# um-dsrg/Super-Resolution-Meta-Attention-Networks

Hardware: AMD Instinct MI355X
Metric: LR-patches/sec (128x128x3, x4) fwd+bwd (higher is better)
Workload: dtype f32

## Files before the change

### super-resolution-meta-attention-networks_amd/csrc/conv3x3_mfma.hip

```cpp
#include "sisr_common.h"
#include "ca_gate.h"
#include <string.h>
#include <stdlib.h>
#include <type_traits>

#define TH 4
#define TW 32
#define HALO_H (TH + 2)
#define HALO_W (TW + 2)
#define HALO_ITEMS (HALO_H * HALO_W * 16)
#define STAGE_ITERS ((HALO_ITEMS + 255) / 256)

struct ConvParams {
  const float* x;
  View xv;
  float* y;
  View yv;
  const float* res;
  const float* mask;
  const float* w;
  const float* bias;
  const float* in_scale;
  const float* in_shift;
  const float* out_scale;
// ... 878 lines not shown
          if (AFFINE) t = t * s4 + t4;
          if (GATE) {
            t = sisr_mul_add4(t, s4, u[r][k]);
            if (rown && cok && col >= 1 && col <= TW)
              sisr_buf_store4(t, ro_, (unsigned)(min(max(gw, 0), W - 1) * (int)p.xv.sW + c4 * 4) * 4u, ro);
          }
          if (!interior) t = sisr_keep_if(t, rok && cok);
          *reinterpret_cast<f32x4*>(lds + r * (HALO_W * 64) + col * 64 + ((c4 ^ (col & 15)) << 2)) = t;
        }
    }
  };

  unsigned aoff[4];
#pragma unroll
  for (int j = 0; j < 4; ++j) {
    const int col = 2 * n + j;
    aoff[j] = (unsigned)(2 * mb * (HALO_W * 64) + col * 64 + ((q ^ (col & 15)) << 2));
  }

  if (t_begin < t_end) {
    halo_regs_t v;
    issue(v, t_begin, 0, HHv);
    commit(v, t_begin);
  }
  __syncthreads();
  for (int tile = t_begin; tile < t_end; tile += t_step) {
    const bool has_next = tile + t_step < t_end;
    int b, h0, w0;
    decode(tile, b, h0, w0);
#define W4_LOAD_B(t) \
  sisr_buf_load4(rw, boff, (unsigned)((((((t) >> 5) * 4 + (((t) >> 1) & 3)) * 4 + (((t) >> 3) & 3)) * 4096) + ((t) & 1) * 256))
    f32x4 bq[8];
#pragma unroll
    for (int t = 0; t < 6; ++t) bq[t] = W4_LOAD_B(t);
    f32x4 y[2][2][2];
    f32x4 acc[4][2];
    f32x4 raw[4], rr[4], av[2][4];
    halo_regs_t v;
    auto read_half = [&](int s, int hc) {
      const int xr = s >> 2, G = s & 3;
      const int ra = xr == 0 ? 0 : (xr == 3 ? 3 : 2), rb = xr == 0 ? 2 : 1;
#pragma unroll
      for (int jj = 0; jj < 2; ++jj) {
        const float* base = lds + (aoff[2 * hc + jj] ^ (unsigned)(G << 4));
        raw[2 * jj] = *reinterpret_cast<const f32x4*>(base + ra * (HALO_W * 64));
        raw[2 * jj + 1] = *reinterpret_cast<const f32x4*>(base + rb * (HALO_W * 64));
      }
    };
    auto rows_half = [&](int s, int hc) {
      const int xr = s >> 2;
#pragma unroll
      for (int jj = 0; jj < 2; ++jj) {
        const f32x4 da = raw[2 * jj], db = raw[2 * jj + 1];
        rr[2 * hc + jj] = xr == 0 ? da - db : (xr == 1 ? db + da : (xr == 2 ? da - db : db - da));
      }
    };
    auto cols_step = [&](int s) {
      f32x4* a = av[s & 1];
      a[0] = rr[0] - rr[2];
      a[1] = rr[1] + rr[2];
      a[2] = rr[2] - rr[1];
      a[3] = rr[1] - rr[3];
    };
    read_half(0, 0);
    rows_half(0, 0);
    read_half(0, 1);
    rows_half(0, 1);
    cols_step(0);
    __builtin_amdgcn_sched_barrier(0);
#pragma unroll
    for (int s = 0; s < 16; ++s) {
      const int xr = s >> 2, G = s & 3;
      if (s == 12 && has_next) issue(v, tile + t_step, 0, 3);
      if (s == 14 && has_next) issue(v, tile + t_step, 3, HHv);
      if (s + 1 < 16) read_half(s + 1, 0);
#pragma unroll
      for (int xc = 0; xc < 4; ++xc) {
        const f32x4 a = av[s & 1][xc];
        f32x4 bb[2];
#pragma unroll
        for (int nb = 0; nb < 2; ++nb) {
          const int t = (s * 4 + xc) * 2 + nb;
          bb[nb] = bq[t & 7];
        }
#pragma unroll
        for (int e = 0; e < 4; ++e)
#pragma unroll
          for (int nb = 0; nb < 2; ++nb) {
            const f32x4 c = (G | e) ? acc[xc][nb] : (f32x4){0.f, 0.f, 0.f, 0.f};
            acc[xc][nb] = __builtin_amdgcn_mfma_f32_16x16x4f32(a[e], bb[nb][e], c, 0, 0, 0);
          }
#pragma unroll
        for (int nb = 0; nb < 2; ++nb) {
          const int t = (s * 4 + xc) * 2 + nb;
          if (t + 6 < 128) bq[(t + 6) & 7] = W4_LOAD_B(t + 6);
        }
        if (s + 1 < 16) {
          if (xc == 1) {
            rows_half(s + 1, 0);
            read_half(s + 1, 1);
          }
          if (xc == 2) rows_half(s + 1, 1);
          if (xc == 3) cols_step(s + 1);
        }
        __builtin_amdgcn_sched_barrier(0);
      }
      if (G == 3) {
#pragma unroll
        for (int nb = 0; nb < 2; ++nb) {
          const f32x4 t0 = acc[0][nb] + acc[1][nb] + acc[2][nb];
          const f32x4 t1 = acc[1][nb] - acc[2][nb] - acc[3][nb];
          if (xr == 0) { y[nb][0][0] = t0; y[nb][0][1] = t1; }
          if (xr == 1) { y[nb][0][0] += t0; y[nb][0][1] += t1; y[nb][1][0] = t0; y[nb][1][1] = t1; }
          if (xr == 2) { y[nb][0][0] += t0; y[nb][0][1] += t1; y[nb][1][0] -= t0; y[nb][1][1] -= t1; }
          if (xr == 3) { y[nb][1][0] -= t0; y[nb][1][1] -= t1; }
#pragma unroll
          for (int i = 0; i < (xr == 0 ? 1 : 2); ++i) asm volatile("" : "+v"(y[nb][i][0]), "+v"(y[nb][i][1]));
        }
      }
    }
#undef W4_LOAD_B
    __syncthreads();
    if (has_next) commit(v, tile + t_step);
    {
      const bool scaled = p.out_scale != nullptr || p.alpha != 1.0f;
      const sisr_rsrc_t ry = sisr_rsrc(p.y + (long)b * p.yv.sB);
      const sisr_rsrc_t rmk = sisr_rsrc(MASK ? p.mask + (long)b * p.yv.sB : p.y);
      const sisr_rsrc_t rrs = sisr_rsrc(RES ? p.res + (long)b * p.yv.sB : p.y);
      const sisr_rsrc_t rdt = sisr_rsrc(DOT ? p.dot + (long)b * p.yv.sB : p.y);
      float gsum[2];
#pragma unroll
      for (int nb = 0; nb < 2; ++nb) {
        const int con = co + 16 * nb;
        float os = p.alpha;
        if (p.out_scale) os *= p.out_scale[(long)b * 64 + con];
        float mk[2][2][4], rs[2][2][4], dt[2][2][4];
#pragma unroll
        for (int i = 0; i < 2; ++i)
#pragma unroll
          for (int j = 0; j < 2; ++j)
#pragma unroll
            for (int r = 0; r < 4; ++r) {
              const int row = min(h0 + 2 * mb + i, H - 1), col = min(w0 + 8 * q + 2 * r + j, W - 1);
              const unsigned vo = (unsigned)(col * (int)p.yv.sW + con) * 4u, so = (unsigned)(row * (int)p.yv.sH) * 4u;
              if (MASK) mk[i][j][r] = sisr_buf_load1(rmk, vo, so);
              if (RES) rs[i][j][r] = sisr_buf_load1(rrs, vo, so);
              if (DOT) dt[i][j][r] = sisr_buf_load1(rdt, vo, so);
            }
        float gs = 0.f;
#pragma unroll
        for (int i = 0; i < 2; ++i)
#pragma unroll
          for (int j = 0; j < 2; ++j)
#pragma unroll
            for (int r = 0; r < 4; ++r) {
              float a = y[nb][i][j][r] + bv[nb];
              if (p.relu) a = fmaxf(a, 0.f);
              if (scaled) a *= os;
              if (MASK) a = mk[i][j][r] > 0.f ? a : 0.f;
              if (RES) a += rs[i][j][r];
              const int row = h0 + 2 * mb + i, col = w0 + 8 * q + 2 * r + j;
              if (row < H && col < W) {
                sisr_buf_store1(a, ry, (unsigned)(col * (int)p.yv.sW + con) * 4u, (unsigned)(row * (int)p.yv.sH) * 4u);
                gs = DOT ? __builtin_fmaf(a, dt[i][j][r], gs) : gs + a;
              }
            }
        gs += __shfl_xor(gs, 16);
        gsum[nb] = gs + __shfl_xor(gs, 32);
      }
      if (p.gap && q == 0) {
        const long parts = (long)p.tiles_w * ((H + 3) / 4) * 2;
        const int th = h0 / THv, tw = w0 / TW;
#pragma unroll
        for (int nb = 0; nb < 2; ++nb) p.gap[(((long)b * parts) + (th * p.tiles_w + tw) * 2 + mb) * 64 + co + 16 * nb] = gsum[nb];
      }
    }
    __syncthreads();
  }
}

typedef __bf16 bf16x8 __attribute__((ext_vector_type(8)));

__device__ __forceinline__ u32x4 sisr_pack_bf16x8(f32x4 a, f32x4 b) {
  bf16x8 r;
  r[0] = (__bf16)a[0]; r[1] = (__bf16)a[1]; r[2] = (__bf16)a[2]; r[3] = (__bf16)a[3];
  r[4] = (__bf16)b[0]; r[5] = (__bf16)b[1]; r[6] = (__bf16)b[2]; r[7] = (__bf16)b[3];
  return __builtin_bit_cast(u32x4, r);
}

__device__ __forceinline__ bf16x8 sisr_buf_load_bf16x8(sisr_rsrc_t r, unsigned voff_bytes, unsigned soff_bytes) {
  return __builtin_bit_cast(bf16x8, __builtin_amdgcn_raw_buffer_load_b128(r, (int)voff_bytes, (int)soff_bytes, 0));
}

#define BH_PIX 128
#define BE_LD 68

template <bool AFFINE, bool MASK, bool RES, bool GATE = false, bool DOT = false>
__global__ __launch_bounds__(256, 3) void conv3x3_c64_bf16_kernel(ConvParams p) {
  extern __shared__ __attribute__((aligned(16))) unsigned char ldsb[];
  const int tid = threadIdx.x, lane = tid & 63, wave = tid >> 6;
  const int q = blockIdx.y;
  int bid;
  {
    const unsigned nb = gridDim.x, xcd = blockIdx.x & 7, idx = blockIdx.x >> 3;
    const unsigned qn = nb >> 3, rn = nb & 7;
    bid = (int)((xcd < rn ? xcd * (qn + 1) : rn * (qn + 1) + (xcd - rn) * qn) + idx);
  }
  const int tw = bid % p.tiles_w;
  bid /= p.tiles_w;
  const int th = bid % p.tiles_h;
  const int b = bid / p.tiles_h;
  const int h0 = th * TH, w0 = tw * TW;
  const int ph = __builtin_amdgcn_readfirstlane(wave >> 1), ch = __builtin_amdgcn_readfirstlane(wave & 1);
  const int n = lane & 31, hh = lane >> 5;
  const int H = p.H, W = p.W;
  const int co = ch * 32 + n;
  const int Cout = p.cout_chunks * 64;

  const float bv = p.bias ? p.bias[co * p.bias_n + q * p.bias_q] : 0.f;
// ... 1853 lines not shown
```

### super-resolution-meta-attention-networks_amd/csrc/diag.hip

```cpp
#include "sisr_common.h"

template <bool RAND>
__global__ __launch_bounds__(256) void mfma_peak_kernel(int iters, float* __restrict__ out,
                                                        unsigned long long* __restrict__ clk) {
  f32x16 acc0 = {0}, acc1 = {0};
  float a = threadIdx.x * 1e-3f, b = 1.0f + blockIdx.x * 1e-6f;
  float ra[4], rb[4];
  if (RAND) {
    unsigned h = (blockIdx.x * 256u + threadIdx.x) * 2654435761u + 12345u;
#pragma unroll
    for (int e = 0; e < 4; ++e) {
      h = h * 1664525u + 1013904223u;
      ra[e] = (float)(int)h * (1.0f / 2147483648.0f);
      h = h * 1664525u + 1013904223u;
      rb[e] = (float)(int)h * (1.0f / 2147483648.0f);
    }
  }
  const unsigned long long t0 = __builtin_amdgcn_s_memtime();
  const unsigned long long r0 = __builtin_amdgcn_s_memrealtime();
  for (int i = 0; i < iters; ++i) {
#pragma unroll
    for (int e = 0; e < 4; ++e) {
      acc0 = __builtin_amdgcn_mfma_f32_32x32x2f32(RAND ? ra[e] : a, RAND ? rb[e] : b, acc0, 0, 0, 0);
      acc1 = __builtin_amdgcn_mfma_f32_32x32x2f32(RAND ? rb[e] : b, RAND ? ra[3 - e] : a, acc1, 0, 0, 0);
    }
    if (!RAND) a += 1e-7f;
  }
  const unsigned long long t1 = __builtin_amdgcn_s_memtime();
  const unsigned long long r1 = __builtin_amdgcn_s_memrealtime();
  float s = 0.f;
#pragma unroll
  for (int r = 0; r < 16; ++r) s += acc0[r] + acc1[r];
  out[(long)blockIdx.x * 256 + threadIdx.x] = s;
  if (blockIdx.x == 0 && threadIdx.x == 0) {
    clk[0] = t1 - t0;
    clk[1] = r1 - r0;
  }
}

extern "C" int sisr_diag_mfma_peak(int blocks, int iters, float* out, unsigned long long* clk, void* stream) {
  if (blocks <= 0 || iters == 0 || !out || !clk) return SISR_ERR_ARG;
  if (iters > 0)
    hipLaunchKernelGGL(mfma_peak_kernel<false>, dim3(blocks), dim3(256), 0, (hipStream_t)stream, iters, out, clk);
  else
    hipLaunchKernelGGL(mfma_peak_kernel<true>, dim3(blocks), dim3(256), 0, (hipStream_t)stream, -iters, out, clk);
  return sisr_check_launch();
}

template <int KIND, int COUNT>
__global__ __launch_bounds__(256) void mfma_fill_kernel(int iters, float* __restrict__ out, const float* __restrict__ src,
                                                        unsigned long long* __restrict__ clk) {
  __shared__ __attribute__((aligned(16))) float lds[256 * 4 + 64];
  f32x16 acc0 = {0}, acc1 = {0};
  float a = threadIdx.x * 1e-3f, b = 1.0f + blockIdx.x * 1e-6f;
  float f0 = a, f1 = b;
  unsigned u0 = threadIdx.x, u1 = blockIdx.x;
  unsigned s0 = blockIdx.x;
  f32x4 q0 = {0.f, 0.f, 0.f, 0.f};
  unsigned long long w0 = threadIdx.x;
  const unsigned lofs = threadIdx.x * 16;
  const float* gp = src + threadIdx.x * 4;
  float* op = out + (long)blockIdx.x * 256 + threadIdx.x;
  lds[threadIdx.x] = a;
  __syncthreads();
  const unsigned long long t0 = __builtin_amdgcn_s_memtime();
  const unsigned long long r0 = __builtin_amdgcn_s_memrealtime();
  for (int i = 0; i < iters; ++i) {
#pragma unroll
    for (int e = 0; e < 8; ++e) {
      if (e & 1) acc1 = __builtin_amdgcn_mfma_f32_32x32x2f32(b, a, acc1, 0, 0, 0);
      else acc0 = __builtin_amdgcn_mfma_f32_32x32x2f32(a, b, acc0, 0, 0, 0);
#pragma unroll
      for (int k = 0; k < (COUNT + 7 - e) / 8; ++k) {
        if (KIND == 1) asm volatile("v_add_f32 %0, %0, %1" : "+v"(f0) : "v"(f1));
        if (KIND == 2) asm volatile("v_and_b32 %0, %0, %1" : "+v"(u0) : "v"(u1));
        if (KIND == 3) asm volatile("s_add_u32 %0, %0, 1" : "+s"(s0) : : "scc");
        if (KIND == 4) asm volatile("ds_read_b128 %0, %1" : "=v"(q0) : "v"(lofs));
        if (KIND == 5) asm volatile("global_load_dwordx4 %0, %1, off" : "=v"(q0) : "v"(gp));
        if (KIND == 6) asm volatile("ds_write_b128 %0, %1" : : "v"(lofs), "v"(q0));
        if (KIND == 7) asm volatile("global_store_dword %0, %1, off" : : "v"(op), "v"(f0));
        if (KIND == 8) asm volatile("v_mov_b32 %0, %1" : "=v"(u0) : "v"(u1));
        if (KIND == 9) asm volatile("s_nop 0");
        if (KIND == 10) asm volatile("v_pk_add_f32 %0, %0, %0" : "+v"(w0));
        if (KIND == 11) asm volatile("v_lshl_add_u64 %0, %0, 0, %0" : "+v"(w0));
        if (KIND == 12) asm volatile("global_load_dwordx4 %0, %1, %2" : "=v"(q0) : "v"(lofs), "s"(src));
      }
    }
    if ((KIND == 4 || KIND == 6) && (i & 3) == 3) asm volatile("s_waitcnt lgkmcnt(0)" ::: "memory");
    if ((KIND == 5 || KIND == 7 || KIND == 12) && (i & 3) == 3 && COUNT <= 8) asm volatile("s_waitcnt vmcnt(0)" ::: "memory");
    if ((KIND == 5 || KIND == 7 || KIND == 12) && (i & 1) == 1 && COUNT == 16) asm volatile("s_waitcnt vmcnt(0)" ::: "memory");
    if ((KIND == 5 || KIND == 7 || KIND == 12) && COUNT == 32) asm volatile("s_waitcnt vmcnt(0)" ::: "memory");
  }
  asm volatile("s_waitcnt vmcnt(0) lgkmcnt(0)" ::: "memory");
  const unsigned long long t1 = __builtin_amdgcn_s_memtime();
  const unsigned long long r1 = __builtin_amdgcn_s_memrealtime();
  float s = f0 + (float)u0 + (float)s0 + q0[0] + q0[3] + (float)(unsigned)w0;
#pragma unroll
  for (int r = 0; r < 16; ++r) s += acc0[r] + acc1[r];
  *op = s;
  if (blockIdx.x == 0 && threadIdx.x == 0) {
    clk[0] = t1 - t0;
    clk[1] = r1 - r0;
  }
}

extern "C" int sisr_diag_mfma_fill(int blocks, int iters, int kind, int count, float* out, const float* src,
                                   unsigned long long* clk, void* stream) {
  if (blocks <= 0 || iters <= 0 || !out || !src || !clk) return SISR_ERR_ARG;
#define FILL(K, C) \
  if (kind == K && count == C) { hipLaunchKernelGGL((mfma_fill_kernel<K, C>), dim3(blocks), dim3(256), 0, (hipStream_t)stream, iters, out, src, clk); return sisr_check_launch(); }
#define FILLK(K) FILL(K, 8) FILL(K, 16) FILL(K, 32)
  FILL(1, 0)
  FILLK(1) FILLK(2) FILLK(3) FILLK(4) FILLK(5) FILLK(6) FILLK(7) FILLK(8) FILLK(9) FILLK(10) FILLK(11) FILLK(12)
#undef FILLK
#undef FILL
  return SISR_ERR_UNSUPPORTED;
}
```

### super-resolution-meta-attention-networks_amd/csrc/sisr_common.h

```cpp
#pragma once
#include <hip/hip_runtime.h>
#include <stdint.h>

typedef float f32x4 __attribute__((ext_vector_type(4)));
typedef float f32x16 __attribute__((ext_vector_type(16)));

struct View {
  long sB, sH, sW;
  long chi, clo;
  int cdiv;
  __host__ __device__ long chunk(int q) const { return (long)(q / cdiv) * chi + (long)(q % cdiv) * clo; }
};

typedef unsigned u32x4 __attribute__((ext_vector_type(4)));
__device__ __forceinline__ f32x4 sisr_keep_if(f32x4 t, bool ok) {
  const unsigned m = ok ? 0xffffffffu : 0u;
  u32x4 b = __builtin_bit_cast(u32x4, t);
  b &= (u32x4){m, m, m, m};
  return __builtin_bit_cast(f32x4, b);
}

__device__ __forceinline__ f32x4 sisr_mul_add4(f32x4 a, f32x4 b, f32x4 c) {
#pragma clang fp contract(off)
  const f32x4 p = a * b;
  return p + c;
}

typedef __amdgpu_buffer_rsrc_t sisr_rsrc_t;
__device__ __forceinline__ sisr_rsrc_t sisr_rsrc(const void* base) {
  return __builtin_amdgcn_make_buffer_rsrc(const_cast<void*>(base), 0, (int)0xffffffffu, 0x00020000);
}
__device__ __forceinline__ f32x4 sisr_buf_load4(sisr_rsrc_t r, unsigned voff_bytes, unsigned soff_bytes) {
  return __builtin_bit_cast(f32x4, __builtin_amdgcn_raw_buffer_load_b128(r, (int)voff_bytes, (int)soff_bytes, 0));
}
__device__ __forceinline__ float sisr_buf_load1(sisr_rsrc_t r, unsigned voff_bytes, unsigned soff_bytes) {
  return __builtin_bit_cast(float, __builtin_amdgcn_raw_buffer_load_b32(r, (int)voff_bytes, (int)soff_bytes, 0));
}
__device__ __forceinline__ void sisr_buf_store4(f32x4 v, sisr_rsrc_t r, unsigned voff_bytes, unsigned soff_bytes) {
  __builtin_amdgcn_raw_buffer_store_b128(__builtin_bit_cast(u32x4, v), r, (int)voff_bytes, (int)soff_bytes, 0);
}
__device__ __forceinline__ void sisr_buf_store1(float v, sisr_rsrc_t r, unsigned voff_bytes, unsigned soff_bytes) {
  __builtin_amdgcn_raw_buffer_store_b32(__builtin_bit_cast(unsigned, v), r, (int)voff_bytes, (int)soff_bytes, 0);
}

#define SISR_OK 0
#define SISR_ERR_ARG (-1)
#define SISR_ERR_ALIGN (-2)
#define SISR_ERR_LAUNCH (-3)
#define SISR_ERR_UNSUPPORTED (-4)

static inline int sisr_check_launch() {
  hipError_t e = hipGetLastError();
  return e == hipSuccess ? SISR_OK : SISR_ERR_LAUNCH - (int)e * 16;
}
#define SISR_ALLOW_LDS(kernel, bytes)                                                                       \
  do {                                                                                                      \
    static bool done_ = false;                                                                              \
    if (!done_) {                                                                                           \
      (void)hipFuncSetAttribute(reinterpret_cast<const void*>(kernel),                                      \
                                hipFuncAttributeMaxDynamicSharedMemorySize, (int)(bytes));                  \
      done_ = true;                                                                                         \
    }                                                                                                       \
  } while (0)

static inline bool sisr_aligned16(const void* p) { return (reinterpret_cast<uintptr_t>(p) & 15) == 0; }
```

### super-resolution-meta-attention-networks_amd/csrc/wgrad3x3_mfma.hip

```cpp
#include "sisr_common.h"
#include <string.h>
#include <stdlib.h>

#define WT_H 8
#define WT_W 32
#define WH_H (WT_H + 2)
#define WH_W (WT_W + 2)
#define WSTR 32
#define X_ITEMS (WH_H * WH_W * 8)
#define X_ITERS ((X_ITEMS + 255) / 256)
#define Y_ITEMS (WT_H * WT_W * 8)
#define Y_ITERS (Y_ITEMS / 256)
#define LDS_X (WH_H * WH_W * WSTR)
#define LDS_Y (WT_H * WT_W * WSTR)
#define SLAB (9 * 16 * 64)
#define WG_MAX_UNITS 64

struct WgradParams {
  const float* x;
  View xv;
  const float* dy;
  View yv;
  const float* dy_scale;
  const float* dy_shift;
// ... 352 lines not shown
            for (int t = 0; t < 9; ++t) an[t] = xn[((t / 3) * WH_W + (t % 3)) * 64];
          }
          __builtin_amdgcn_sched_barrier(0);
#pragma unroll
          for (int t = 0; t < 9; ++t) acc[t] = __builtin_amdgcn_mfma_f32_32x32x2f32(av[t], bv, acc[t], 0, 0, 0);
          __builtin_amdgcn_sched_barrier(0);
          bv = bn;
#pragma unroll
          for (int t = 0; t < 9; ++t) av[t] = an[t];
        }
        xa = xn;
        yb = yn;
      }
    }
    __syncthreads();
    if (has_next) {
      commit(tile + t_step);
      __syncthreads();
    }
  }

  {
    float* out = p.slabs + ((long)blockIdx.x * ((long)gridDim.y * 4) + pair * 4 + cih * 2 + coh) * SLAB;
#pragma unroll
    for (int t = 0; t < 9; ++t)
#pragma unroll
      for (int r = 0; r < 16; ++r) out[(t * 16 + r) * 64 + lane] = acc[t][r];
  }
  if (do_bias) {
    __syncthreads();
    float* red = lds;
    *reinterpret_cast<f32x4*>(red + tid * 8) = bsa;
    *reinterpret_cast<f32x4*>(red + tid * 8 + 4) = bsb;
    __syncthreads();
    if (tid < 64) {
      const int cc8 = tid >> 3, e = tid & 7;
      float s = 0.f;
      for (int k = 0; k < 32; ++k) s += red[(k * 8 + cc8) * 8 + e];
      p.bias_slabs[((long)blockIdx.x * p.cout_chunks + cq) * 64 + tid] = s;
    }
  }
}

__global__ __launch_bounds__(256, 1) void wgrad3x3_c64_full_kernel(WgradParams p) { wgrad3x3_c64_full_body(p); }
__global__ __launch_bounds__(256, 1) void wgrad3x3_c64_full_batch_kernel(WgradBatch bt) { wgrad3x3_c64_full_body(bt.job[blockIdx.z]); }
__global__ __launch_bounds__(256, 1) void wgrad3x3_c64_full_geo_kernel(WgradParams p) { wgrad3x3_c64_full_body<true>(p); }

#define W4_TH 4
#define W4_HH (W4_TH + 2)
#define W4G_X (W4_HH * WH_W * 64)
#define W4G_Y (W4_TH * WT_W * 64)
#define W4G_LDS ((W4G_X + W4G_Y) * 4)

__global__ __launch_bounds__(256, 1) void wgrad3x3_c64_w4_kernel(WgradParams p) {
  extern __shared__ __attribute__((aligned(16))) float lds[];
  float* const ldx = lds;
  float* const ldy = lds + W4G_X;
  const int tid = threadIdx.x, lane = tid & 63, wave = tid >> 6;
  const int pair = blockIdx.y;
  const int cq = pair % p.cout_chunks, cc = pair / p.cout_chunks;
  const int cih = __builtin_amdgcn_readfirstlane(wave >> 1), coh = __builtin_amdgcn_readfirstlane(wave & 1);
  const int i = lane & 31, kk = lane >> 5;
  const int H = p.H, W = p.W;
  const bool do_bias = p.bias_slabs && cc == 0;
  const bool affine = p.dy_scale != nullptr || p.dy_shift != nullptr;
  const int Cout = p.cout_chunks * 64;

  f32x16 acc[16];
#pragma unroll
  for (int t = 0; t < 16; ++t) acc[t] = (f32x16){0};
  f32x4 bsa = {0.f, 0.f, 0.f, 0.f}, bsb = bsa;

  const int tiles_w = p.tiles_w, tiles_h = (H + W4_TH - 1) / W4_TH;
  const int tiles_per_img = tiles_w * tiles_h;
  const int total = tiles_per_img * p.B;
  int t_begin = blockIdx.x, t_end = total, t_step = p.S;
  if ((p.S & 7) == 0) {
    const int xcd = blockIdx.x & 7, idx = blockIdx.x >> 3, per = (total + 7) >> 3;
    t_begin = xcd * per + idx;
    t_end = min(total, (xcd + 1) * per);
    t_step = p.S >> 3;
  }
  struct Stage {
    f32x4 x[W4_HH][2];
    f32x4 xe[2];
    f32x4 y[W4_TH][2];
  };
  Stage st;
  const int c8 = tid & 7, pcol = tid >> 3;
  const int eidx = tid % 96, er = eidx >> 4, eside = (eidx >> 3) & 1, ec8 = eidx & 7;
  auto decode = [&](int tile, int& b, int& h0, int& w0) {
    b = tile / tiles_per_img;
    const int tr = tile - b * tiles_per_img;
    const int th = tr / tiles_w;
    h0 = th * W4_TH;
    w0 = (tr - th * tiles_w) * WT_W;
  };
  auto issue = [&](int tile) {
    int b, h0, w0;
    decode(tile, b, h0, w0);
    const sisr_rsrc_t rx = sisr_rsrc(p.x + (long)b * p.xv.sB + p.xv.chunk(cc));
    const sisr_rsrc_t ry = sisr_rsrc(p.dy + (long)b * p.yv.sB + p.yv.chunk(cq));
    const unsigned vx = (unsigned)(min(w0 + pcol, W - 1) * (int)p.xv.sW + c8 * 8) * 4u;
    const unsigned vy = (unsigned)(min(w0 + pcol, W - 1) * (int)p.yv.sW + c8 * 8) * 4u;
#pragma unroll
    for (int r = 0; r < W4_HH; ++r) {
      const unsigned so = (unsigned)(min(max(h0 - 1 + r, 0), H - 1) * (int)p.xv.sH) * 4u;
      st.x[r][0] = sisr_buf_load4(rx, vx, so);
      st.x[r][1] = sisr_buf_load4(rx, vx + 16u, so);
    }
    {
      const int gwe = min(max(eside ? w0 + WT_W : w0 - 1, 0), W - 1);
      const unsigned ve = (unsigned)(min(max(h0 - 1 + er, 0), H - 1) * (int)p.xv.sH + gwe * (int)p.xv.sW + ec8 * 8) * 4u;
      st.xe[0] = sisr_buf_load4(rx, ve, 0u);
      st.xe[1] = sisr_buf_load4(rx, ve + 16u, 0u);
    }
#pragma unroll
    for (int r = 0; r < W4_TH; ++r) {
      const unsigned so = (unsigned)(min(h0 + r, H - 1) * (int)p.yv.sH) * 4u;
      st.y[r][0] = sisr_buf_load4(ry, vy, so);
      st.y[r][1] = sisr_buf_load4(ry, vy + 16u, so);
    }
  };
  auto commit = [&](int tile) {
    int b, h0, w0;
    decode(tile, b, h0, w0);
    const bool interior = h0 >= 1 && h0 + W4_TH + 1 <= H && w0 >= 1 && w0 + WT_W + 1 <= W;
    const bool okc = w0 + pcol < W;
    if (!interior) {
#pragma unroll
      for (int r = 0; r < W4_HH; ++r) {
        const int gh = h0 - 1 + r;
        const bool ok = gh >= 0 && gh < H && okc;
        st.x[r][0] = sisr_keep_if(st.x[r][0], ok);
        st.x[r][1] = sisr_keep_if(st.x[r][1], ok);
      }
      const int gwe = eside ? w0 + WT_W : w0 - 1, ghe = h0 - 1 + er;
      const bool oke = ghe >= 0 && ghe < H && gwe >= 0 && gwe < W;
      st.xe[0] = sisr_keep_if(st.xe[0], oke);
      st.xe[1] = sisr_keep_if(st.xe[1], oke);
    }
    float* lx = ldx + (pcol + 1) * 64 + c8 * 8;
#pragma unroll
    for (int r = 0; r < W4_HH; ++r) {
      *reinterpret_cast<f32x4*>(lx + r * (WH_W * 64)) = st.x[r][0];
      *reinterpret_cast<f32x4*>(lx + r * (WH_W * 64) + 4) = st.x[r][1];
    }
    if (tid < 96) {
      float* le = ldx + (er * WH_W + (eside ? WH_W - 1 : 0)) * 64 + ec8 * 8;
      *reinterpret_cast<f32x4*>(le) = st.xe[0];
      *reinterpret_cast<f32x4*>(le + 4) = st.xe[1];
    }
    if (affine) {
      f32x4 s4a = {1.f, 1.f, 1.f, 1.f}, s4b = s4a, t4a = {0.f, 0.f, 0.f, 0.f}, t4b = t4a;
      if (p.dy_scale) {
        const float* sp = p.dy_scale + (long)b * Cout + cq * 64 + c8 * 8;
        s4a = *reinterpret_cast<const f32x4*>(sp);
        s4b = *reinterpret_cast<const f32x4*>(sp + 4);
      }
      if (p.dy_shift) {
        const float* tp = p.dy_shift + (long)b * Cout + cq * 64 + c8 * 8;
        t4a = *reinterpret_cast<const f32x4*>(tp);
        t4b = *reinterpret_cast<const f32x4*>(tp + 4);
      }
#pragma unroll
      for (int r = 0; r < W4_TH; ++r) {
        st.y[r][0] = st.y[r][0] * s4a + t4a;
        st.y[r][1] = st.y[r][1] * s4b + t4b;
      }
    }
    if (!interior) {
#pragma unroll
      for (int r = 0; r < W4_TH; ++r) {
        const bool ok = okc && h0 + r < H;
        st.y[r][0] = sisr_keep_if(st.y[r][0], ok);
        st.y[r][1] = sisr_keep_if(st.y[r][1], ok);
      }
    }
    float* ly = ldy + pcol * 64 + c8 * 8;
#pragma unroll
    for (int r = 0; r < W4_TH; ++r) {
      *reinterpret_cast<f32x4*>(ly + r * (WT_W * 64)) = st.y[r][0];
      *reinterpret_cast<f32x4*>(ly + r * (WT_W * 64) + 4) = st.y[r][1];
    }
    if (do_bias) {
#pragma unroll
      for (int r = 0; r < W4_TH; ++r) {
        bsa += st.y[r][0];
        bsb += st.y[r][1];
      }
    }
  };

  const float* const xl = ldx + kk * (2 * 64) + cih * 32 + i;
  const float* const yl = ldy + kk * (2 * 64) + coh * 32 + i;
  struct Raw {
    float d[4][4], y[2][2];
  };
  auto fetch = [&](int ks, Raw& rw) {
    const int br = ks >> 3, bc = ks & 7;
#pragma unroll
    for (int r = 0; r < 4; ++r)
#pragma unroll
      for (int j = 0; j < 4; ++j) rw.d[r][j] = xl[((2 * br + r) * WH_W + 4 * bc + j) * 64];
#pragma unroll
    for (int r = 0; r < 2; ++r)
#pragma unroll
      for (int j = 0; j < 2; ++j) rw.y[r][j] = yl[((2 * br + r) * WT_W + 4 * bc + j) * 64];
  };
  auto transform = [&](const Raw& rw, float (&V)[16], float (&M)[16]) {
    float rr[4][4];
#pragma unroll
    for (int j = 0; j < 4; ++j) {
      rr[0][j] = rw.d[0][j] - rw.d[2][j];
      rr[1][j] = rw.d[1][j] + rw.d[2][j];
      rr[2][j] = rw.d[2][j] - rw.d[1][j];
      rr[3][j] = rw.d[1][j] - rw.d[3][j];
    }
#pragma unroll
    for (int xr = 0; xr < 4; ++xr) {
      V[xr * 4 + 0] = rr[xr][0] - rr[xr][2];
      V[xr * 4 + 1] = rr[xr][1] + rr[xr][2];
      V[xr * 4 + 2] = rr[xr][2] - rr[xr][1];
      V[xr * 4 + 3] = rr[xr][1] - rr[xr][3];
    }
    float ry[4][2];
#pragma unroll
    for (int j = 0; j < 2; ++j) {
      ry[0][j] = rw.y[0][j];
      ry[1][j] = rw.y[0][j] + rw.y[1][j];
      ry[2][j] = rw.y[0][j] - rw.y[1][j];
      ry[3][j] = rw.y[1][j];
    }
#pragma unroll
    for (int xr = 0; xr < 4; ++xr) {
      M[xr * 4 + 0] = ry[xr][0];
      M[xr * 4 + 1] = ry[xr][0] + ry[xr][1];
      M[xr * 4 + 2] = ry[xr][0] - ry[xr][1];
      M[xr * 4 + 3] = ry[xr][1];
    }
  };

  float V[2][16], M[2][16];
  auto step_order = [&]() {
#pragma unroll
    for (int t = 0; t < 2; ++t) {
      __builtin_amdgcn_sched_group_barrier(0x008, 1, 0);
      __builtin_amdgcn_sched_group_barrier(0x100, 5, 0);
    }
    __builtin_amdgcn_sched_group_barrier(0x008, 2, 0);
#pragma unroll
    for (int t = 4; t < 15; ++t) {
      __builtin_amdgcn_sched_group_barrier(0x008, 1, 0);
      __builtin_amdgcn_sched_group_barrier(0x002, 4, 0);
    }
    __builtin_amdgcn_sched_group_barrier(0x008, 1, 0);
  };
  if (t_begin < t_end) {
    issue(t_begin);
    commit(t_begin);
    __syncthreads();
    Raw rw;
    fetch(0, rw);
    transform(rw, V[0], M[0]);
  }
  for (int tile = t_begin; tile < t_end; tile += t_step) {
    const bool has_next = tile + t_step < t_end;
    if (has_next) issue(tile + t_step);
#pragma unroll
    for (int ks = 0; ks < 15; ++ks) {
      const int cur = ks & 1, nxt = cur ^ 1;
      Raw rw;
      fetch(ks + 1, rw);
#pragma unroll
      for (int t = 0; t < 16; ++t)
        acc[t] = __builtin_amdgcn_mfma_f32_32x32x2f32(V[cur][t], M[cur][t], acc[t], 0, 0, 0);
      transform(rw, V[nxt], M[nxt]);
      step_order();
    }
    __syncthreads();
    if (has_next) commit(tile + t_step);
#pragma unroll
    for (int t = 0; t < 8; ++t) acc[t] = __builtin_amdgcn_mfma_f32_32x32x2f32(V[1][t], M[1][t], acc[t], 0, 0, 0);
    __builtin_amdgcn_sched_barrier(0);
    __syncthreads();
    {
      Raw rw;
      fetch(0, rw);
#pragma unroll
      for (int t = 8; t < 16; ++t) acc[t] = __builtin_amdgcn_mfma_f32_32x32x2f32(V[1][t], M[1][t], acc[t], 0, 0, 0);
      transform(rw, V[0], M[0]);
      __builtin_amdgcn_sched_group_barrier(0x008, 1, 0);
      __builtin_amdgcn_sched_group_barrier(0x100, 10, 0);
      __builtin_amdgcn_sched_group_barrier(0x008, 2, 0);
#pragma unroll
      for (int t = 0; t < 5; ++t) {
        __builtin_amdgcn_sched_group_barrier(0x008, 1, 0);
        __builtin_amdgcn_sched_group_barrier(0x002, 9, 0);
      }
    }
  }

  {
    float* out = p.slabs + ((long)blockIdx.x * ((long)gridDim.y * 4) + pair * 4 + cih * 2 + coh) * SLAB;
    auto fold = [](float u0, float u1, float u2, float u3, float& f0, float& f1, float& f2) {
      const float h = 0.5f * (u1 + u2);
      f0 = u0 + h;
      f1 = 0.5f * (u1 - u2);
      f2 = h - u3;
    };
#pragma unroll
    for (int r = 0; r < 16; ++r) {
      float rw[3][4];
#pragma unroll
      for (int xc = 0; xc < 4; ++xc) fold(acc[xc][r], acc[4 + xc][r], acc[8 + xc][r], acc[12 + xc][r], rw[0][xc], rw[1][xc], rw[2][xc]);
#pragma unroll
      for (int kh = 0; kh < 3; ++kh) {
        float g0, g1, g2;
        fold(rw[kh][0], rw[kh][1], rw[kh][2], rw[kh][3], g0, g1, g2);
        out[((kh * 3 + 0) * 16 + r) * 64 + lane] = g0;
        out[((kh * 3 + 1) * 16 + r) * 64 + lane] = g1;
        out[((kh * 3 + 2) * 16 + r) * 64 + lane] = g2;
      }
    }
  }
  if (do_bias) {
    __syncthreads();
    float* red = lds;
    *reinterpret_cast<f32x4*>(red + tid * 8) = bsa;
    *reinterpret_cast<f32x4*>(red + tid * 8 + 4) = bsb;
    __syncthreads();
    if (tid < 64) {
      const int cc8 = tid >> 3, e = tid & 7;
      float s = 0.f;
      for (int k = 0; k < 32; ++k) s += red[(k * 8 + cc8) * 8 + e];
      p.bias_slabs[((long)blockIdx.x * p.cout_chunks + cq) * 64 + tid] = s;
    }
  }
}

typedef __bf16 bf16x4 __attribute__((ext_vector_type(4)));
typedef __bf16 bf16x8 __attribute__((ext_vector_type(8)));
typedef bf16x4 __attribute__((address_space(3))) * lds_bf16x4_ptr;
#define BW_PIX 128
#define BW_X_BYTES (WH_H * WH_W * BW_PIX)
#define BW_Y_BYTES (WT_H * WT_W * BW_PIX)

__device__ __forceinline__ u32x4 wg_pack_bf16x8(f32x4 a, f32x4 b) {
  bf16x8 r;
  r[0] = (__bf16)a[0]; r[1] = (__bf16)a[1]; r[2] = (__bf16)a[2]; r[3] = (__bf16)a[3];
  r[4] = (__bf16)b[0]; r[5] = (__bf16)b[1]; r[6] = (__bf16)b[2]; r[7] = (__bf16)b[3];
  return __builtin_bit_cast(u32x4, r);
}

__device__ __forceinline__ bf16x8 wg_tr_frag(const unsigned char* base, unsigned off0, unsigned off1) {
  const bf16x4 lo = __builtin_amdgcn_ds_read_tr16_b64_v4bf16((lds_bf16x4_ptr)(base + off0));
  const bf16x4 hi = __builtin_amdgcn_ds_read_tr16_b64_v4bf16((lds_bf16x4_ptr)(base + off1));
  return __builtin_shufflevector(lo, hi, 0, 1, 2, 3, 4, 5, 6, 7);
}

template <bool X16, bool Y16>
static __device__ __forceinline__ void wgrad3x3_c64_bf16_body(const WgradParams& p, unsigned* stamp = nullptr) {
  extern __shared__ __attribute__((aligned(16))) unsigned char ldsb[];
  unsigned char* ldx = ldsb;
  unsigned char* ldy = ldsb + BW_X_BYTES;
  const int tid = threadIdx.x, lane = tid & 63, wave = tid >> 6;
  const int pair = blockIdx.y;
  const int cq = pair % p.cout_chunks, cc = pair / p.cout_chunks;
  const int cih = __builtin_amdgcn_readfirstlane(wave >> 1), coh = __builtin_amdgcn_readfirstlane(wave & 1);
  const int H = p.H, W = p.W;
  const bool do_bias = p.bias_slabs && cc == 0;
  const int Cout = p.cout_chunks * 64;

  f32x16 acc[9];
#pragma unroll
  for (int t = 0; t < 9; ++t) acc[t] = (f32x16){0};
  f32x4 bsa = {0.f, 0.f, 0.f, 0.f}, bsb = bsa;

  unsigned aoff[3][2], yoff[2];
  {
    const int g = lane >> 4, qq = (lane >> 2) & 3, pp = lane & 3;
    const int chunk = (g & 1) * 2 + (pp >> 1), sub = (pp & 1) * 8;
#pragma unroll
    for (int rd = 0; rd < 2; ++rd) {
      const int pix = 8 * (g >> 1) + 4 * rd + qq;
      yoff[rd] = pix * BW_PIX + (((coh * 4 + chunk) ^ (((pix >> 1) & 1) << 2)) << 4) + sub;
// ... 1104 lines not shown
```

Baseline: 119.2.

## Use packed v_pk_add_f32 for Winograd transforms and reschedule wgrad interleaving

Replaces scalar f32 add/sub in the conv3x3 Winograd input and output transforms with packed v_pk_add_f32 inline asm, halving the VALU instruction count. The wgrad kernel's input transform is rewritten on f32x2 pairs using op_sel/neg modifiers, and explicit sched barriers interleave the transform ops between individual MFMAs. The channel-to-thread mapping of the global and LDS staging changes to strided halves, with the bias reduction indexing updated to match. Diagnostic microbenchmarks for packed-add throughput alongside MFMA are added. Inline asm volatile may constrain compiler scheduling, and the remapping risks correctness errors if any index is missed.

After: 123.5, median of 6. +3.6%, better.

```diff
diff --git a/super-resolution-meta-attention-networks_amd/csrc/conv3x3_mfma.hip b/super-resolution-meta-attention-networks_amd/csrc/conv3x3_mfma.hip
--- a/super-resolution-meta-attention-networks_amd/csrc/conv3x3_mfma.hip
+++ b/super-resolution-meta-attention-networks_amd/csrc/conv3x3_mfma.hip
@@ -954,15 +954,15 @@
 #pragma unroll
       for (int jj = 0; jj < 2; ++jj) {
         const f32x4 da = raw[2 * jj], db = raw[2 * jj + 1];
-        rr[2 * hc + jj] = xr == 0 ? da - db : (xr == 1 ? db + da : (xr == 2 ? da - db : db - da));
+        rr[2 * hc + jj] = xr == 0 ? sisr_pk4_sub(da, db) : (xr == 1 ? sisr_pk4_add(db, da) : (xr == 2 ? sisr_pk4_sub(da, db) : sisr_pk4_sub(db, da)));
       }
     };
     auto cols_step = [&](int s) {
       f32x4* a = av[s & 1];
-      a[0] = rr[0] - rr[2];
-      a[1] = rr[1] + rr[2];
-      a[2] = rr[2] - rr[1];
-      a[3] = rr[1] - rr[3];
+      a[0] = sisr_pk4_sub(rr[0], rr[2]);
+      a[1] = sisr_pk4_add(rr[1], rr[2]);
+      a[2] = sisr_pk4_sub(rr[2], rr[1]);
+      a[3] = sisr_pk4_sub(rr[1], rr[3]);
     };
     read_half(0, 0);
     rows_half(0, 0);
@@ -1008,14 +1008,19 @@
         __builtin_amdgcn_sched_barrier(0);
       }
       if (G == 3) {
+        f32x4 t0[2], t1[2];
+#pragma unroll
+        for (int nb = 0; nb < 2; ++nb) t0[nb] = sisr_pk4_add(sisr_pk4_add(acc[0][nb], acc[1][nb]), acc[2][nb]);
+#pragma unroll
+        for (int nb = 0; nb < 2; ++nb) t1[nb] = sisr_pk4_sub(acc[1][nb], acc[2][nb]);
+#pragma unroll
+        for (int nb = 0; nb < 2; ++nb) t1[nb] = sisr_pk4_sub(t1[nb], acc[3][nb]);
 #pragma unroll
         for (int nb = 0; nb < 2; ++nb) {
-          const f32x4 t0 = acc[0][nb] + acc[1][nb] + acc[2][nb];
-          const f32x4 t1 = acc[1][nb] - acc[2][nb] - acc[3][nb];
-          if (xr == 0) { y[nb][0][0] = t0; y[nb][0][1] = t1; }
-          if (xr == 1) { y[nb][0][0] += t0; y[nb][0][1] += t1; y[nb][1][0] = t0; y[nb][1][1] = t1; }
-          if (xr == 2) { y[nb][0][0] += t0; y[nb][0][1] += t1; y[nb][1][0] -= t0; y[nb][1][1] -= t1; }
-          if (xr == 3) { y[nb][1][0] -= t0; y[nb][1][1] -= t1; }
+          if (xr == 0) { y[nb][0][0] = t0[nb]; y[nb][0][1] = t1[nb]; }
+          if (xr == 1 || xr == 2) { y[nb][0][0] = sisr_pk4_add(y[nb][0][0], t0[nb]); y[nb][0][1] = sisr_pk4_add(y[nb][0][1], t1[nb]); }
+          if (xr == 1) { y[nb][1][0] = t0[nb]; y[nb][1][1] = t1[nb]; }
+          if (xr >= 2) { y[nb][1][0] = sisr_pk4_sub(y[nb][1][0], t0[nb]); y[nb][1][1] = sisr_pk4_sub(y[nb][1][1], t1[nb]); }
 #pragma unroll
           for (int i = 0; i < (xr == 0 ? 1 : 2); ++i) asm volatile("" : "+v"(y[nb][i][0]), "+v"(y[nb][i][1]));
         }
@@ -1050,13 +1055,15 @@
               if (DOT) dt[i][j][r] = sisr_buf_load1(rdt, vo, so);
             }
         float gs = 0.f;
+        const f32x4 bv4 = {bv[nb], bv[nb], bv[nb], bv[nb]};
 #pragma unroll
         for (int i = 0; i < 2; ++i)
 #pragma unroll
-          for (int j = 0; j < 2; ++j)
+          for (int j = 0; j < 2; ++j) {
+            const f32x4 yb = sisr_pk4_add(y[nb][i][j], bv4);
 #pragma unroll
             for (int r = 0; r < 4; ++r) {
-              float a = y[nb][i][j][r] + bv[nb];
+              float a = yb[r];
               if (p.relu) a = fmaxf(a, 0.f);
               if (scaled) a *= os;
               if (MASK) a = mk[i][j][r] > 0.f ? a : 0.f;
@@ -1067,6 +1074,7 @@
                 gs = DOT ? __builtin_fmaf(a, dt[i][j][r], gs) : gs + a;
               }
             }
+          }
         gs += __shfl_xor(gs, 16);
         gsum[nb] = gs + __shfl_xor(gs, 32);
       }
diff --git a/super-resolution-meta-attention-networks_amd/csrc/diag.hip b/super-resolution-meta-attention-networks_amd/csrc/diag.hip
--- a/super-resolution-meta-attention-networks_amd/csrc/diag.hip
+++ b/super-resolution-meta-attention-networks_amd/csrc/diag.hip
@@ -47,11 +47,12 @@
   return sisr_check_launch();
 }
 
-template <int KIND, int COUNT>
+template <int KIND, int COUNT, int MF = 0>
 __global__ __launch_bounds__(256) void mfma_fill_kernel(int iters, float* __restrict__ out, const float* __restrict__ src,
                                                         unsigned long long* __restrict__ clk) {
   __shared__ __attribute__((aligned(16))) float lds[256 * 4 + 64];
   f32x16 acc0 = {0}, acc1 = {0};
+  f32x4 c4[4] = {{0.f, 0.f, 0.f, 0.f}, {0.f, 0.f, 0.f, 0.f}, {0.f, 0.f, 0.f, 0.f}, {0.f, 0.f, 0.f, 0.f}};
   float a = threadIdx.x * 1e-3f, b = 1.0f + blockIdx.x * 1e-6f;
   float f0 = a, f1 = b;
   unsigned u0 = threadIdx.x, u1 = blockIdx.x;
@@ -68,7 +69,8 @@
   for (int i = 0; i < iters; ++i) {
 #pragma unroll
     for (int e = 0; e < 8; ++e) {
-      if (e & 1) acc1 = __builtin_amdgcn_mfma_f32_32x32x2f32(b, a, acc1, 0, 0, 0);
+      if (MF == 1) c4[e & 3] = __builtin_amdgcn_mfma_f32_16x16x4f32(e & 1 ? b : a, e & 1 ? a : b, c4[e & 3], 0, 0, 0);
+      else if (e & 1) acc1 = __builtin_amdgcn_mfma_f32_32x32x2f32(b, a, acc1, 0, 0, 0);
       else acc0 = __builtin_amdgcn_mfma_f32_32x32x2f32(a, b, acc0, 0, 0, 0);
 #pragma unroll
       for (int k = 0; k < (COUNT + 7 - e) / 8; ++k) {
@@ -84,6 +86,8 @@
         if (KIND == 10) asm volatile("v_pk_add_f32 %0, %0, %0" : "+v"(w0));
         if (KIND == 11) asm volatile("v_lshl_add_u64 %0, %0, 0, %0" : "+v"(w0));
         if (KIND == 12) asm volatile("global_load_dwordx4 %0, %1, %2" : "=v"(q0) : "v"(lofs), "s"(src));
+        if (KIND == 13) asm volatile("v_pk_add_f32 %0, %0, %0 neg_lo:[0,1] neg_hi:[0,1]" : "+v"(w0));
+        if (KIND == 14) asm volatile("v_pk_add_f32 %0, %0, %0 op_sel:[1,0] op_sel_hi:[1,1] neg_lo:[0,1] neg_hi:[0,1]" : "+v"(w0));
       }
     }
     if ((KIND == 4 || KIND == 6) && (i & 3) == 3) asm volatile("s_waitcnt lgkmcnt(0)" ::: "memory");
@@ -97,6 +101,8 @@
   float s = f0 + (float)u0 + (float)s0 + q0[0] + q0[3] + (float)(unsigned)w0;
 #pragma unroll
   for (int r = 0; r < 16; ++r) s += acc0[r] + acc1[r];
+#pragma unroll
+  for (int r = 0; r < 4; ++r) s += c4[r][0] + c4[r][1] + c4[r][2] + c4[r][3];
   *op = s;
   if (blockIdx.x == 0 && threadIdx.x == 0) {
     clk[0] = t1 - t0;
@@ -107,11 +113,14 @@
 extern "C" int sisr_diag_mfma_fill(int blocks, int iters, int kind, int count, float* out, const float* src,
                                    unsigned long long* clk, void* stream) {
   if (blocks <= 0 || iters <= 0 || !out || !src || !clk) return SISR_ERR_ARG;
-#define FILL(K, C) \
-  if (kind == K && count == C) { hipLaunchKernelGGL((mfma_fill_kernel<K, C>), dim3(blocks), dim3(256), 0, (hipStream_t)stream, iters, out, src, clk); return sisr_check_launch(); }
-#define FILLK(K) FILL(K, 8) FILL(K, 16) FILL(K, 32)
-  FILL(1, 0)
-  FILLK(1) FILLK(2) FILLK(3) FILLK(4) FILLK(5) FILLK(6) FILLK(7) FILLK(8) FILLK(9) FILLK(10) FILLK(11) FILLK(12)
+#define FILL(K, C, MF) \
+  if (kind == K + 100 * MF && count == C) { hipLaunchKernelGGL((mfma_fill_kernel<K, C, MF>), dim3(blocks), dim3(256), 0, (hipStream_t)stream, iters, out, src, clk); return sisr_check_launch(); }
+#define FILLK(K) FILL(K, 8, 0) FILL(K, 16, 0) FILL(K, 32, 0)
+#define FILLA(K) FILL(K, 5, 0) FILL(K, 10, 0) FILL(K, 11, 0) FILL(K, 22, 0) FILL(K, 5, 1) FILL(K, 8, 1) FILL(K, 10, 1) FILL(K, 11, 1) FILL(K, 16, 1) FILL(K, 22, 1)
+  FILL(1, 0, 0) FILL(1, 0, 1)
+  FILLK(1) FILLK(2) FILLK(3) FILLK(4) FILLK(5) FILLK(6) FILLK(7) FILLK(8) FILLK(9) FILLK(10) FILLK(11) FILLK(12) FILLK(13) FILLK(14)
+  FILLA(1) FILLA(10) FILLA(13) FILLA(14)
+#undef FILLA
 #undef FILLK
 #undef FILL
   return SISR_ERR_UNSUPPORTED;
diff --git a/super-resolution-meta-attention-networks_amd/csrc/sisr_common.h b/super-resolution-meta-attention-networks_amd/csrc/sisr_common.h
--- a/super-resolution-meta-attention-networks_amd/csrc/sisr_common.h
+++ b/super-resolution-meta-attention-networks_amd/csrc/sisr_common.h
@@ -24,6 +24,26 @@
 #pragma clang fp contract(off)
   const f32x4 p = a * b;
   return p + c;
+}
+
+typedef float f32x2 __attribute__((ext_vector_type(2)));
+__device__ __forceinline__ f32x2 sisr_pk_add(f32x2 a, f32x2 b) {
+  f32x2 r;
+  asm volatile("v_pk_add_f32 %0, %1, %2" : "=v"(r) : "v"(a), "v"(b));
+  return r;
+}
+__device__ __forceinline__ f32x2 sisr_pk_sub(f32x2 a, f32x2 b) {
+  f32x2 r;
+  asm volatile("v_pk_add_f32 %0, %1, %2 neg_lo:[0,1] neg_hi:[0,1]" : "=v"(r) : "v"(a), "v"(b));
+  return r;
+}
+__device__ __forceinline__ f32x4 sisr_pk4_add(f32x4 a, f32x4 b) {
+  const f32x2 lo = sisr_pk_add(a.xy, b.xy), hi = sisr_pk_add(a.zw, b.zw);
+  return (f32x4){lo.x, lo.y, hi.x, hi.y};
+}
+__device__ __forceinline__ f32x4 sisr_pk4_sub(f32x4 a, f32x4 b) {
+  const f32x2 lo = sisr_pk_sub(a.xy, b.xy), hi = sisr_pk_sub(a.zw, b.zw);
+  return (f32x4){lo.x, lo.y, hi.x, hi.y};
 }
 
 typedef __amdgpu_buffer_rsrc_t sisr_rsrc_t;
diff --git a/super-resolution-meta-attention-networks_amd/csrc/wgrad3x3_mfma.hip b/super-resolution-meta-attention-networks_amd/csrc/wgrad3x3_mfma.hip
--- a/super-resolution-meta-attention-networks_amd/csrc/wgrad3x3_mfma.hip
+++ b/super-resolution-meta-attention-networks_amd/csrc/wgrad3x3_mfma.hip
@@ -428,6 +428,22 @@
 #define W4G_Y (W4_TH * WT_W * 64)
 #define W4G_LDS ((W4G_X + W4G_Y) * 4)
 
+__device__ __forceinline__ f32x2 pk_add_nl(f32x2 a, f32x2 b) {
+  f32x2 r;
+  asm volatile("v_pk_add_f32 %0, %1, %2 op_sel_hi:[1,0] neg_lo:[0,1]" : "=v"(r) : "v"(a), "v"(b));
+  return r;
+}
+__device__ __forceinline__ f32x2 pk_hh_sub(f32x2 a, f32x2 b) {
+  f32x2 r;
+  asm volatile("v_pk_add_f32 %0, %1, %2 op_sel:[1,0] op_sel_hi:[1,1] neg_lo:[0,1] neg_hi:[0,1]" : "=v"(r) : "v"(a), "v"(b));
+  return r;
+}
+__device__ __forceinline__ f32x2 pk_h_pm_l(f32x2 a) {
+  f32x2 r;
+  asm volatile("v_pk_add_f32 %0, %1, %1 op_sel:[1,0] op_sel_hi:[1,0] neg_hi:[0,1]" : "=v"(r) : "v"(a));
+  return r;
+}
+
 __global__ __launch_bounds__(256, 1) void wgrad3x3_c64_w4_kernel(WgradParams p) {
   extern __shared__ __attribute__((aligned(16))) float lds[];
   float* const ldx = lds;
@@ -477,25 +493,25 @@
     decode(tile, b, h0, w0);
     const sisr_rsrc_t rx = sisr_rsrc(p.x + (long)b * p.xv.sB + p.xv.chunk(cc));
     const sisr_rsrc_t ry = sisr_rsrc(p.dy + (long)b * p.yv.sB + p.yv.chunk(cq));
-    const unsigned vx = (unsigned)(min(w0 + pcol, W - 1) * (int)p.xv.sW + c8 * 8) * 4u;
-    const unsigned vy = (unsigned)(min(w0 + pcol, W - 1) * (int)p.yv.sW + c8 * 8) * 4u;
+    const unsigned vx = (unsigned)(min(w0 + pcol, W - 1) * (int)p.xv.sW + c8 * 4) * 4u;
+    const unsigned vy = (unsigned)(min(w0 + pcol, W - 1) * (int)p.yv.sW + c8 * 4) * 4u;
 #pragma unroll
     for (int r = 0; r < W4_HH; ++r) {
       const unsigned so = (unsigned)(min(max(h0 - 1 + r, 0), H - 1) * (int)p.xv.sH) * 4u;
       st.x[r][0] = sisr_buf_load4(rx, vx, so);
-      st.x[r][1] = sisr_buf_load4(rx, vx + 16u, so);
+      st.x[r][1] = sisr_buf_load4(rx, vx + 128u, so);
     }
     {
       const int gwe = min(max(eside ? w0 + WT_W : w0 - 1, 0), W - 1);
-      const unsigned ve = (unsigned)(min(max(h0 - 1 + er, 0), H - 1) * (int)p.xv.sH + gwe * (int)p.xv.sW + ec8 * 8) * 4u;
+      const unsigned ve = (unsigned)(min(max(h0 - 1 + er, 0), H - 1) * (int)p.xv.sH + gwe * (int)p.xv.sW + ec8 * 4) * 4u;
       st.xe[0] = sisr_buf_load4(rx, ve, 0u);
-      st.xe[1] = sisr_buf_load4(rx, ve + 16u, 0u);
+      st.xe[1] = sisr_buf_load4(rx, ve + 128u, 0u);
     }
 #pragma unroll
     for (int r = 0; r < W4_TH; ++r) {
       const unsigned so = (unsigned)(min(h0 + r, H - 1) * (int)p.yv.sH) * 4u;
       st.y[r][0] = sisr_buf_load4(ry, vy, so);
-      st.y[r][1] = sisr_buf_load4(ry, vy + 16u, so);
+      st.y[r][1] = sisr_buf_load4(ry, vy + 128u, so);
     }
   };
   auto commit = [&](int tile) {
@@ -516,28 +532,28 @@
       st.xe[0] = sisr_keep_if(st.xe[0], oke);
       st.xe[1] = sisr_keep_if(st.xe[1], oke);
     }
-    float* lx = ldx + (pcol + 1) * 64 + c8 * 8;
+    float* lx = ldx + (pcol + 1) * 64 + c8 * 4;
 #pragma unroll
     for (int r = 0; r < W4_HH; ++r) {
       *reinterpret_cast<f32x4*>(lx + r * (WH_W * 64)) = st.x[r][0];
-      *reinterpret_cast<f32x4*>(lx + r * (WH_W * 64) + 4) = st.x[r][1];
+      *reinterpret_cast<f32x4*>(lx + r * (WH_W * 64) + 32) = st.x[r][1];
     }
     if (tid < 96) {
-      float* le = ldx + (er * WH_W + (eside ? WH_W - 1 : 0)) * 64 + ec8 * 8;
+      float* le = ldx + (er * WH_W + (eside ? WH_W - 1 : 0)) * 64 + ec8 * 4;
       *reinterpret_cast<f32x4*>(le) = st.xe[0];
-      *reinterpret_cast<f32x4*>(le + 4) = st.xe[1];
+      *reinterpret_cast<f32x4*>(le + 32) = st.xe[1];
     }
     if (affine) {
       f32x4 s4a = {1.f, 1.f, 1.f, 1.f}, s4b = s4a, t4a = {0.f, 0.f, 0.f, 0.f}, t4b = t4a;
       if (p.dy_scale) {
-        const float* sp = p.dy_scale + (long)b * Cout + cq * 64 + c8 * 8;
+        const float* sp = p.dy_scale + (long)b * Cout + cq * 64 + c8 * 4;
         s4a = *reinterpret_cast<const f32x4*>(sp);
-        s4b = *reinterpret_cast<const f32x4*>(sp + 4);
+        s4b = *reinterpret_cast<const f32x4*>(sp + 32);
       }
       if (p.dy_shift) {
-        const float* tp = p.dy_shift + (long)b * Cout + cq * 64 + c8 * 8;
+        const float* tp = p.dy_shift + (long)b * Cout + cq * 64 + c8 * 4;
         t4a = *reinterpret_cast<const f32x4*>(tp);
-        t4b = *reinterpret_cast<const f32x4*>(tp + 4);
+        t4b = *reinterpret_cast<const f32x4*>(tp + 32);
       }
 #pragma unroll
       for (int r = 0; r < W4_TH; ++r) {
@@ -553,11 +569,11 @@
         st.y[r][1] = sisr_keep_if(st.y[r][1], ok);
       }
     }
-    float* ly = ldy + pcol * 64 + c8 * 8;
+    float* ly = ldy + pcol * 64 + c8 * 4;
 #pragma unroll
     for (int r = 0; r < W4_TH; ++r) {
       *reinterpret_cast<f32x4*>(ly + r * (WT_W * 64)) = st.y[r][0];
-      *reinterpret_cast<f32x4*>(ly + r * (WT_W * 64) + 4) = st.y[r][1];
+      *reinterpret_cast<f32x4*>(ly + r * (WT_W * 64) + 32) = st.y[r][1];
     }
     if (do_bias) {
 #pragma unroll
@@ -571,74 +587,62 @@
   const float* const xl = ldx + kk * (2 * 64) + cih * 32 + i;
   const float* const yl = ldy + kk * (2 * 64) + coh * 32 + i;
   struct Raw {
-    float d[4][4], y[2][2];
+    f32x2 d[4][2], y[2];
   };
   auto fetch = [&](int ks, Raw& rw) {
     const int br = ks >> 3, bc = ks & 7;
 #pragma unroll
-    for (int r = 0; r < 4; ++r)
-#pragma unroll
-      for (int j = 0; j < 4; ++j) rw.d[r][j] = xl[((2 * br + r) * WH_W + 4 * bc + j) * 64];
-#pragma unroll
-    for (int r = 0; r < 2; ++r)
-#pragma unroll
-      for (int j = 0; j < 2; ++j) rw.y[r][j] = yl[((2 * br + r) * WT_W + 4 * bc + j) * 64];
-  };
-  auto transform = [&](const Raw& rw, float (&V)[16], float (&M)[16]) {
-    float rr[4][4];
-#pragma unroll
-    for (int j = 0; j < 4; ++j) {
-      rr[0][j] = rw.d[0][j] - rw.d[2][j];
-      rr[1][j] = rw.d[1][j] + rw.d[2][j];
-      rr[2][j] = rw.d[2][j] - rw.d[1][j];
-      rr[3][j] = rw.d[1][j] - rw.d[3][j];
-    }
-#pragma unroll
-    for (int xr = 0; xr < 4; ++xr) {
-      V[xr * 4 + 0] = rr[xr][0] - rr[xr][2];
-      V[xr * 4 + 1] = rr[xr][1] + rr[xr][2];
-      V[xr * 4 + 2] = rr[xr][2] - rr[xr][1];
-      V[xr * 4 + 3] = rr[xr][1] - rr[xr][3];
-    }
-    float ry[4][2];
-#pragma unroll
-    for (int j = 0; j < 2; ++j) {
-      ry[0][j] = rw.y[0][j];
-      ry[1][j] = rw.y[0][j] + rw.y[1][j];
-      ry[2][j] = rw.y[0][j] - rw.y[1][j];
-      ry[3][j] = rw.y[1][j];
-    }
-#pragma unroll
-    for (int xr = 0; xr < 4; ++xr) {
-      M[xr * 4 + 0] = ry[xr][0];
-      M[xr * 4 + 1] = ry[xr][0] + ry[xr][1];
-      M[xr * 4 + 2] = ry[xr][0] - ry[xr][1];
-      M[xr * 4 + 3] = ry[xr][1];
-    }
-  };
-
-  float V[2][16], M[2][16];
-  auto step_order = [&]() {
-#pragma unroll
-    for (int t = 0; t < 2; ++t) {
-      __builtin_amdgcn_sched_group_barrier(0x008, 1, 0);
-      __builtin_amdgcn_sched_group_barrier(0x100, 5, 0);
-    }
-    __builtin_amdgcn_sched_group_barrier(0x008, 2, 0);
-#pragma unroll
-    for (int t = 4; t < 15; ++t) {
-      __builtin_amdgcn_sched_group_barrier(0x008, 1, 0);
-      __builtin_amdgcn_sched_group_barrier(0x002, 4, 0);
-    }
-    __builtin_amdgcn_sched_group_barrier(0x008, 1, 0);
-  };
+    for (int c = 0; c < 2; ++c)
+#pragma unroll
+      for (int r = 0; r < 4; ++r) {
+        const float* q = xl + ((2 * br + r) * WH_W + 4 * bc + 2 * c) * 64;
+        rw.d[r][c] = (f32x2){q[0], q[64]};
+      }
+#pragma unroll
+    for (int r = 0; r < 2; ++r) {
+      const float* q = yl + ((2 * br + r) * WT_W + 4 * bc) * 64;
+      rw.y[r] = (f32x2){q[0], q[64]};
+    }
+  };
+  struct Ops {
+    f32x2 va[4], vb[4], ry[4], mc[4];
+  };
+  f32x2 rr[4][2];
+  auto transform_op = [&](int k, const Raw& rw, Ops& o) {
+    if (k < 8) {
+      const int c = k >> 2, r = k & 3;
+      rr[r][c] = r == 0 ? sisr_pk_sub(rw.d[0][c], rw.d[2][c]) : r == 1 ? sisr_pk_add(rw.d[1][c], rw.d[2][c])
+               : r == 2 ? sisr_pk_sub(rw.d[2][c], rw.d[1][c]) : sisr_pk_sub(rw.d[1][c], rw.d[3][c]);
+    } else if (k < 16) {
+      const int xr = (k - 8) >> 1;
+      if (k & 1) o.vb[xr] = pk_hh_sub(rr[xr][0], rr[xr][1]);
+      else o.va[xr] = pk_add_nl(rr[xr][0], rr[xr][1]);
+    } else if (k == 16) {
+      o.ry[0] = rw.y[0];
+      o.ry[3] = rw.y[1];
+      o.ry[1] = sisr_pk_add(rw.y[0], rw.y[1]);
+    } else if (k == 17) {
+      o.ry[2] = sisr_pk_sub(rw.y[0], rw.y[1]);
+    } else {
+      o.mc[k - 18] = pk_h_pm_l(o.ry[k - 18]);
+    }
+  };
+  auto mfma = [&](int t, const Ops& o) {
+    const int xr = t >> 2, xc = t & 3;
+    const float a = xc == 0 ? o.va[xr].x : xc == 1 ? o.va[xr].y : xc == 2 ? o.vb[xr].x : o.vb[xr].y;
+    const float b = xc == 0 ? o.ry[xr].x : xc == 1 ? o.mc[xr].x : xc == 2 ? o.mc[xr].y : o.ry[xr].y;
+    acc[t] = __builtin_amdgcn_mfma_f32_32x32x2f32(a, b, acc[t], 0, 0, 0);
+  };
+
+  Ops ops[2];
   if (t_begin < t_end) {
     issue(t_begin);
     commit(t_begin);
     __syncthreads();
     Raw rw;
     fetch(0, rw);
-    transform(rw, V[0], M[0]);
+#pragma unroll
+    for (int k = 0; k < 22; ++k) transform_op(k, rw, ops[0]);
   }
   for (int tile = t_begin; tile < t_end; tile += t_step) {
     const bool has_next = tile + t_step < t_end;
@@ -647,33 +651,49 @@
     for (int ks = 0; ks < 15; ++ks) {
       const int cur = ks & 1, nxt = cur ^ 1;
       Raw rw;
+      __builtin_amdgcn_sched_barrier(0);
+      mfma(0, ops[cur]);
+      __builtin_amdgcn_sched_barrier(0);
       fetch(ks + 1, rw);
-#pragma unroll
-      for (int t = 0; t < 16; ++t)
-        acc[t] = __builtin_amdgcn_mfma_f32_32x32x2f32(V[cur][t], M[cur][t], acc[t], 0, 0, 0);
-      transform(rw, V[nxt], M[nxt]);
-      step_order();
+      __builtin_amdgcn_sched_barrier(0);
+#pragma unroll
+      for (int t = 1; t < 4; ++t) mfma(t, ops[cur]);
+#pragma unroll
+      for (int t = 4; t < 15; ++t) {
+        __builtin_amdgcn_sched_barrier(0);
+        mfma(t, ops[cur]);
+        __builtin_amdgcn_sched_barrier(0);
+        transform_op(2 * (t - 4), rw, ops[nxt]);
+        transform_op(2 * (t - 4) + 1, rw, ops[nxt]);
+      }
+      __builtin_amdgcn_sched_barrier(0);
+      mfma(15, ops[cur]);
+      __builtin_amdgcn_sched_barrier(0);
     }
     __syncthreads();
     if (has_next) commit(tile + t_step);
 #pragma unroll
-    for (int t = 0; t < 8; ++t) acc[t] = __builtin_amdgcn_mfma_f32_32x32x2f32(V[1][t], M[1][t], acc[t], 0, 0, 0);
+    for (int t = 0; t < 8; ++t) mfma(t, ops[1]);
     __builtin_amdgcn_sched_barrier(0);
     __syncthreads();
     {
       Raw rw;
+      mfma(8, ops[1]);
+      __builtin_amdgcn_sched_barrier(0);
       fetch(0, rw);
-#pragma unroll
-      for (int t = 8; t < 16; ++t) acc[t] = __builtin_amdgcn_mfma_f32_32x32x2f32(V[1][t], M[1][t], acc[t], 0, 0, 0);
-      transform(rw, V[0], M[0]);
-      __builtin_amdgcn_sched_group_barrier(0x008, 1, 0);
-      __builtin_amdgcn_sched_group_barrier(0x100, 10, 0);
-      __builtin_amdgcn_sched_group_barrier(0x008, 2, 0);
-#pragma unroll
-      for (int t = 0; t < 5; ++t) {
-        __builtin_amdgcn_sched_group_barrier(0x008, 1, 0);
-        __builtin_amdgcn_sched_group_barrier(0x002, 9, 0);
-      }
+      __builtin_amdgcn_sched_barrier(0);
+      mfma(9, ops[1]);
+      mfma(10, ops[1]);
+#pragma unroll
+      for (int t = 11; t < 16; ++t) {
+        const int k0 = t < 13 ? 5 * (t - 11) : 10 + 4 * (t - 13), k1 = t < 13 ? k0 + 5 : k0 + 4;
+        __builtin_amdgcn_sched_barrier(0);
+#pragma unroll
+        for (int k = k0; k < k1; ++k) transform_op(k, rw, ops[0]);
+        __builtin_amdgcn_sched_barrier(0);
+        mfma(t, ops[1]);
+      }
+      __builtin_amdgcn_sched_barrier(0);
     }
   }
 
@@ -707,7 +727,7 @@
     *reinterpret_cast<f32x4*>(red + tid * 8 + 4) = bsb;
     __syncthreads();
     if (tid < 64) {
-      const int cc8 = tid >> 3, e = tid & 7;
+      const int cc8 = (tid & 31) >> 2, e = (tid & 3) + 4 * (tid >> 5);
       float s = 0.f;
       for (int k = 0; k < 32; ++k) s += red[(k * 8 + cc8) * 8 + e];
       p.bias_slabs[((long)blockIdx.x * p.cout_chunks + cq) * 64 + tid] = s;
```
